# slp-rl/aero

Hardware: NVIDIA H100
Metric: audio-seconds/sec forward (higher is better)
Workload: dtype f16 tensor-core operands and activation storage (10-bit mantissa = tf32), fp32 accumulate / norm inputs / cell state

## Files before the change

aero_b200/cabi.py:

```python
from __future__ import annotations

import ctypes as C
import os

_HERE = os.path.dirname(os.path.abspath(__file__))
LIB_PATH = os.path.join(_HERE, "libaero_b200.so")

i32, i64, f32 = C.c_int32, C.c_int64, C.c_float
vp = C.c_void_p


class StftParams(C.Structure):
    _fields_ = [("n_fft", i32), ("hop", i32), ("win", i32), ("n_signals", i32), ("channels", i32),
                ("length", i32), ("frames", i32), ("bins_out", i32),
                ("z_stride_b", i64), ("z_stride_c", i64), ("z_stride_k", i64), ("z_stride_t", i64),
                ("flags", i32), ("reserved", i32)]


class IstftParams(C.Structure):
    _fields_ = [("n_fft", i32), ("hop", i32), ("win", i32), ("n_signals", i32), ("channels", i32),
                ("frames", i32), ("bins_in", i32), ("out_len", i32),
                ("z_stride_b", i64), ("z_stride_c", i64), ("z_stride_k", i64), ("z_stride_t", i64),
                ("flags", i32), ("reserved", i32)]

# ... 34 lines not shown

class ResampleParams(C.Structure):
    _fields_ = [("B", i32), ("C", i32), ("L_in", i32), ("orig", i32), ("up", i32), ("width", i32), ("taps", i32),
                ("L_hr", i32), ("L_valid", i32), ("halo", i32), ("fill", i32), ("normalize", i32), ("floor_", f32)]


ABI_VERSION = 3
TAPS_CONV, TAPS_CONVT, TAPS_MIX = 0, 1, 2
ACT_NONE, ACT_GELU, ACT_RELU, ACT_LEAKY, ACT_TANH = 0, 1, 2, 3, 4
TG_ROUND_TF32, TG_A_F16, TG_OUT_F16, TG_REVERSE = 1, 2, 4, 8
NA_NONE, NA_GELU, NA_GLU, NA_SNAKE, NA_GLU_SCALE_RES, NA_RELU, NA_LEAKY, NA_TANH = 0, 1, 2, 3, 4, 5, 6, 7
NA_NO_NORM = 16
STFT_ZERO_PAD, STFT_ADJ_SCALE, ISTFT_RAW = 1, 2, 1

SYMBOLS = {
    "aero_abi_version": (C.c_int, []),
    "aero_last_error": (C.c_char_p, []),
    "aero_device_arch": (C.c_int, []),
    "aero_launch_count": (C.c_uint64, []),
    "aero_stft_fwd": (C.c_int, [vp, vp, vp, vp, C.POINTER(StftParams), vp]),
    "aero_istft_fwd": (C.c_int, [vp, vp, vp, C.POINTER(IstftParams), vp]),
    "aero_tapgemm_fwd": (C.c_int, [vp] * 10 + [C.POINTER(TapGemmParams), vp]),
    "aero_tapgemm_tc_eligible": (C.c_int, [C.POINTER(TapGemmParams)]),
    "aero_sample_norm_fwd": (C.c_int, [vp, vp, vp, vp, i32, i64, i64, i32, vp]),
    "aero_norm_act_fwd": (C.c_int, [vp] * 8 + [C.POINTER(NormActParams), vp]),
    "aero_ftb_lin_out_fwd": (C.c_int, [vp] * 7 + [C.POINTER(FtbLinParams), vp]),
    "aero_ftb_lin_squeeze_fwd": (C.c_int, [vp, vp, vp, vp, i32, C.POINTER(FtbLinParams), vp]),
    "aero_freq_mix_small_fwd": (C.c_int, [vp, vp, vp, vp, i32, i32, i64, i32, vp]),
    "aero_lstm_rec_fwd": (C.c_int, [vp, vp, vp, vp, C.POINTER(LstmParams), vp]),
    "aero_local_attn_fwd": (C.c_int, [vp, vp, C.POINTER(AttnParams), vp]),
    "aero_lsd_fwd": (C.c_int, [vp, vp, vp, i32, i32, i32, i32, vp]),
    "aero_stft_loss_fwd": (C.c_int, [vp, vp, vp, i32, i32, i32, i32, vp]),
    "aero_stft_loss_bwd": (C.c_int, [vp, vp, vp, vp, i32, i32, i32, i32, f32, f32, vp]),
    "aero_tapgemm_wgrad": (C.c_int, [vp, vp, vp, vp, C.POINTER(TapGemmParams), i64, i64, i64, vp]),
    "aero_colsum": (C.c_int, [vp, vp, vp, vp, i32, i32, i64, i64, i64, i64, i32, i64, i64, vp]),
    "aero_add": (C.c_int, [vp, vp, i64, f32, vp]),
    "aero_add_f64": (C.c_int, [vp, vp, i64, vp]),
    "aero_gram": (C.c_int, [vp, vp, vp, vp, i32, i32, i64, i64, i64, i64, vp]),
    "aero_bcast_add": (C.c_int, [vp, vp, i32, i32, i32, i32, vp]),
    "aero_scale_rows": (C.c_int, [vp, vp, vp, i32, i64, i32, vp]),
    "aero_norm_act_train_fwd": (C.c_int, [vp] * 8 + [C.POINTER(NormActParams), vp]),
    "aero_norm_act_train_bwd": (C.c_int, [vp] * 13 + [i32, C.POINTER(NormActParams), vp]),
    "aero_adam_step": (C.c_int, [vp, i32, f32, f32, f32, f32, i32, f32, vp]),
    "aero_pack_kmajor_tf32": (C.c_int, [vp, vp, vp, i32, i32, i32, vp]),
    "aero_split_tf32": (C.c_int, [vp, vp, vp, i64, vp]),
    "aero_tapgemm_wgrad_tc_eligible": (C.c_int, [C.POINTER(TapGemmParams), vp, vp, vp]),
# ... 57 lines not shown
```

aero_b200/csrc/tapgemm_tc.cu:

```cuda
#include <cuda.h>
#include <mutex>
#include <unordered_map>
#include <string>
#include <cstring>
#include <cstdlib>

#include "tapgemm.cuh"
#include "tc_common.cuh"

namespace aero {

KernelFn tapgemm_tc_kernels_bn32(bool f16a, bool f16o, int amode, bool res, bool stats);
KernelFn tapgemm_tc_kernels_bn64(bool f16a, bool f16o, int amode, bool res, bool stats);
KernelFn tapgemm_tc_kernels_bn96(bool f16a, bool f16o, int amode, bool res, bool stats);
KernelFn tapgemm_tc_kernels_bn128(bool f16a, bool f16o, int amode, bool res, bool stats);

typedef CUresult (*EncodeTiledFn)(CUtensorMap*, CUtensorMapDataType, cuuint32_t, void*, const cuuint64_t*, const cuuint64_t*,
                                  const cuuint32_t*, const cuuint32_t*, CUtensorMapInterleave, CUtensorMapSwizzle,
                                  CUtensorMapL2promotion, CUtensorMapFloatOOBfill);

static EncodeTiledFn get_encode() {
    static EncodeTiledFn fn = nullptr;
    static std::once_flag once;
    std::call_once(once, [] {
        void* p = nullptr;
        cudaDriverEntryPointQueryResult qres;
        if (cudaGetDriverEntryPoint("cuTensorMapEncodeTiled", &p, cudaEnableDefault, &qres) == cudaSuccess &&
            qres == cudaDriverEntryPointSuccess)
            fn = reinterpret_cast<EncodeTiledFn>(p);
    });
    return fn;
}

struct MapKey {
    const void* base;
    uint64_t d[4], s[3];
    uint32_t box[4], rank, swz, pad_;
    bool operator==(const MapKey& o) const { return std::memcmp(this, &o, sizeof(MapKey)) == 0; }
// ... 67 lines not shown
        return p.w_sb == 0 && p.C1 % q == 0 && p.C2 == 0 && p.a1_st % q == 0 && p.a1_sb % q == 0 && p.N >= 8 &&
               p.stats_mode == 0 && !p.glu && p.F_out == 1 && p.F_in == 1 && tc_stages(p.N, pick_bn(p.N)) >= 2;
    if (p.w_sb != 0) return false;
    if (p.act == AERO_ACT_TANH) return false;
    if (p.act == AERO_ACT_LEAKY && (p.stats_mode != 0 || p.r_sb != 0 || p.r_sf != 0 || p.r_st != 0))
        return false;
    if (tc_stages(p.N, pick_bn(p.N)) < 2) return false;
    if (p.N < 8) return false;
    const int K = p.C1 + p.C2;
    if (K < 8 || (p.C1 % q) || (p.C2 % q)) return false;
    auto ok_strides = [q](int64_t sb, int64_t sf, int64_t st) { return sb % q == 0 && sf % q == 0 && st % q == 0 && st > 0; };
    if (p.C1 && !ok_strides(p.a1_sb, p.a1_sf, p.a1_st)) return false;
    if (p.C2 && !ok_strides(p.a2_sb, p.a2_sf, p.a2_st)) return false;
    if (p.stats_mode == 1) {
        const int Nout = p.glu ? p.N / 2 : p.N;
        if (p.groups < 1 || Nout % p.groups) return false;
        const int gw = Nout / p.groups;
        const int bn = pick_bn(p.N);
        if (gw % 8 || (p.glu ? bn / 2 : bn) / gw + 2 > 8) return false;
    }
    return true;
}

static int make_a_map(CUtensorMap* m, const void* base, int C, const aero_tapgemm_params& p, int64_t sb, int64_t sf, int64_t st, int esz) {
    uint64_t dims[4] = {(uint64_t)C, (uint64_t)p.T_in, (uint64_t)p.F_in, (uint64_t)p.B};
    int64_t s1 = st, s2 = sf, s3 = sb;
    if (s2 <= 0) s2 = s1 * p.T_in;
    if (s3 <= 0) s3 = s2 * p.F_in;
    uint64_t strides[3] = {(uint64_t)s1 * esz, (uint64_t)s2 * esz, (uint64_t)s3 * esz};
    uint32_t box[4] = {(uint32_t)(128 / esz), (uint32_t)kBM, 1, 1};
    return encode_map(m, base, 4, dims, strides, box, 0, esz);
}

struct TcKnobs {
    int direct_f32 = -1, direct_f16 = -1, stages = -1;
    TcKnobs() {
        auto rd = [](const char* name, int& v) { if (const char* e = getenv(name)) v = atoi(e); };
        rd("AERO_TC_DIRECT_F32", direct_f32); rd("AERO_TC_DIRECT_F16", direct_f16); rd("AERO_TC_STAGES", stages);
    }
};
static const TcKnobs& knobs() { static const TcKnobs k; return k; }

int tapgemm_tc_launch(const TapGemmArgs& g0, cudaStream_t st) {
    const TcKnobs& kn = knobs();
    TapGemmArgs g = g0;
    const aero_tapgemm_params& p = g.p;
    const bool f16a = p.precision == 2, f16o = (p.flags & AERO_TG_OUT_F16) != 0;
    const int esz = f16a ? 2 : 4, kBKc = 128 / esz;
    const int K = p.C1 + p.C2;
    const int BN = pick_bn(p.N);
    const int nslab = (p.mode == AERO_TAPS_CONVT) ? p.kf : p.kf * p.kt;
    CUtensorMap mA1, mA2, mW;
    int rc;
    const bool mix = p.mode == AERO_TAPS_MIX;
    if (mix) {
        uint64_t dims[3] = {(uint64_t)p.T, (uint64_t)p.C1, (uint64_t)p.B};
        uint64_t strides[2] = {(uint64_t)p.a1_st * esz, (uint64_t)(p.a1_sb > 0 ? p.a1_sb : (int64_t)p.a1_st * p.C1) * esz};
        uint32_t box[3] = {(uint32_t)(f16a ? 64 : 32), (uint32_t)kBKc, 1};
        if ((rc = encode_map(&mA1, g.a1, 3, dims, strides, box, 0, esz)) != AERO_OK) return rc;
    } else if (p.C1) { if ((rc = make_a_map(&mA1, g.a1, p.C1, p, p.a1_sb, p.a1_sf, p.a1_st, esz)) != AERO_OK) return rc; }
    if (p.C2) { if ((rc = make_a_map(&mA2, g.a2, p.C2, p, p.a2_sb, p.a2_sf, p.a2_st, esz)) != AERO_OK) return rc; }
    if (!p.C1) mA1 = mA2;
    if (!p.C2) mA2 = mA1;
    {
        const uint64_t npad = (uint64_t)((p.N + 3) & ~3);
        const uint64_t kp = f16a ? (uint64_t)((K + 7) & ~7) : (uint64_t)K;
        uint64_t dims[3] = {(uint64_t)K, npad, (uint64_t)nslab};
        uint64_t strides[2] = {kp * esz, kp * npad * esz};
        uint32_t box[3] = {(uint32_t)kBKc, (uint32_t)BN, 1};
        if ((rc = encode_map(&mW, g.w, 3, dims, strides, box, 0, esz)) != AERO_OK) return rc;
    }
    g.tiles_t = cdiv(p.T, kBM);
    g.direct_f32 = 0;
    g.direct_f16 = 2;
    if (kn.direct_f32 >= 0) g.direct_f32 = kn.direct_f32;
    if (kn.direct_f16 >= 0) g.direct_f16 = kn.direct_f16;
    const int64_t tiles = (int64_t)p.B * p.F_out * g.tiles_t;
    if (tiles > 2147483647LL) { set_error("aero_tapgemm_fwd: too many tiles"); return AERO_ERR_INVALID; }
    {
        const uint32_t divs[3] = {(uint32_t)cdiv(p.N, BN), (uint32_t)g.tiles_t, (uint32_t)p.F_out};
        for (int i = 0; i < 3; ++i) {
            uint32_t s = 0;
            while ((1ull << s) < divs[i]) ++s;
            const uint64_t two = 1ull << (31 + s);
            g.dv_mul[i] = (uint32_t)((two + divs[i] - 1) / divs[i]);
            g.dv_shr[i] = 31 + s;
        }
    }
    const int stage_bytes = kATileBytes + BN * 128;
    const int fixed = tc_fixed_smem(p.N, BN);
    int kStages = tc_stages(p.N, BN);
    if (kStages < 2) {
        set_error("aero_tapgemm_fwd(wgmma): N = %d leaves no shared memory for the pipeline", p.N);
        return AERO_ERR_UNSUPPORTED;
    }
    if (kn.stages >= 2 && kn.stages < kStages) kStages = kn.stages;
    const size_t smem = (size_t)kStages * stage_bytes + fixed;
    const int amode = p.glu ? 3 : (p.act == AERO_ACT_LEAKY ? 4 : p.act);
    if (p.glu && p.act != AERO_ACT_NONE) { set_error("aero_tapgemm_fwd(wgmma): GLU with an activation is not supported"); return AERO_ERR_UNSUPPORTED; }
    const bool res = g.residual != nullptr, stats = p.stats_mode != 0;
    const KernelFn kern = BN == 32 ? tapgemm_tc_kernels_bn32(f16a, f16o, amode, res, stats)
                        : BN == 64 ? tapgemm_tc_kernels_bn64(f16a, f16o, amode, res, stats)
                        : BN == 96 ? tapgemm_tc_kernels_bn96(f16a, f16o, amode, res, stats)
                                   : tapgemm_tc_kernels_bn128(f16a, f16o, amode, res, stats);
    if (!kern) {
        set_error("aero_tapgemm_fwd(wgmma): epilogue (act %d, residual %d, stats %d) is not built for operands %s / outputs %s",
                  amode, (int)res, (int)stats, f16a ? "f16" : "tf32", f16o ? "f16" : "f32");
        return AERO_ERR_UNSUPPORTED;
    }
    cudaFuncSetAttribute(kern, cudaFuncAttributeMaxDynamicSharedMemorySize, 227 * 1024);
    static int num_sms = 0;
    if (num_sms == 0) {
        int dev = 0;
        cudaGetDevice(&dev);
        cudaDeviceGetAttribute(&num_sms, cudaDevAttrMultiProcessorCount, dev);
    }
    const int n_tiles = cdiv(p.N, BN);
    const int64_t tiles_total = tiles * n_tiles;
    if (tiles_total > 2147483647LL) { set_error("aero_tapgemm_fwd: too many tiles"); return AERO_ERR_INVALID; }
    const int64_t want = num_sms;
    g.last_tile = (int)tiles_total - 1;
    dim3 grid((unsigned)(tiles_total < want ? tiles_total : want));
    kern<<<grid, kThreads, smem, st>>>(mA1, mA2, mW, g, kStages, n_tiles, (int)tiles_total);
    return check_launch("aero_tapgemm_fwd(wgmma)");
}

}
```

aero_b200/csrc/tapgemm_tc_bn128.cu:

```cuda
#include "tapgemm_tc_kernel.cuh"

namespace aero {
KernelFn tapgemm_tc_kernels_bn128(bool f16a, bool f16o, int amode, bool res, bool stats) { return pick_kernel_bn<128>(f16a, f16o, amode, res, stats); }
}
```

aero_b200/csrc/tapgemm_tc_bn32.cu:

```cuda
#include "tapgemm_tc_kernel.cuh"

namespace aero {
KernelFn tapgemm_tc_kernels_bn32(bool f16a, bool f16o, int amode, bool res, bool stats) { return pick_kernel_bn<32>(f16a, f16o, amode, res, stats); }
}
```

aero_b200/csrc/tapgemm_tc_bn64.cu:

```cuda
#include "tapgemm_tc_kernel.cuh"

namespace aero {
KernelFn tapgemm_tc_kernels_bn64(bool f16a, bool f16o, int amode, bool res, bool stats) { return pick_kernel_bn<64>(f16a, f16o, amode, res, stats); }
}
```

aero_b200/csrc/tapgemm_tc_bn96.cu:

```cuda
#include "tapgemm_tc_kernel.cuh"

namespace aero {
KernelFn tapgemm_tc_kernels_bn96(bool f16a, bool f16o, int amode, bool res, bool stats) { return pick_kernel_bn<96>(f16a, f16o, amode, res, stats); }
}
```

aero_b200/csrc/tapgemm_tc_kernel.cuh:

```cuda
#pragma once
#include <cuda.h>
#include <type_traits>

#include "tapgemm.cuh"
#include "tc_common.cuh"


namespace aero {

template <bool F16A> struct OperandKind { static constexpr int kBK = F16A ? 64 : 32; };

struct TapIter {
    int fi, dt, slab;
};
__device__ __forceinline__ bool tap_geometry(const aero_tapgemm_params& p, int tap, int fo, TapIter& it) {
    if (p.mode == AERO_TAPS_CONV) {
        const int jf = tap / p.kt, jt = tap - jf * p.kt;
        it.fi = fo * p.stride_f + jf - p.pad_f;
        it.dt = jt * p.dil_t - p.pad_t;
        it.slab = tap;
    } else {
        const int fof = fo + p.f_out_offset;
        it.fi = fof / p.stride_f - tap;
        it.dt = 0;
        it.slab = fof % p.stride_f + tap * p.stride_f;
    }
    return it.fi >= 0 && it.fi < p.F_in;
}

struct TileCoord {
    int b, fo, t0, n0, n_iters;
};
__device__ __forceinline__ int fast_div(int n, uint32_t mul, uint32_t shr) {
    return (int)(((uint64_t)(uint32_t)n * mul) >> shr);
}
__device__ __forceinline__ int valid_taps(const aero_tapgemm_params& p, int fo, int ntaps) {
    if (p.mode == AERO_TAPS_CONV) {
        const int base = fo * p.stride_f - p.pad_f;
        const int lo = max(0, -base), hi = min(p.kf - 1, p.F_in - 1 - base);
        return max(0, hi - lo + 1) * p.kt;
    }
    const int a = (fo + p.f_out_offset) / p.stride_f;
    const int lo = max(0, a - p.F_in + 1), hi = min(ntaps - 1, a);
    return max(0, hi - lo + 1);
}
__device__ __forceinline__ TileCoord tile_coord(const TapGemmArgs& g, int tile, int n_tiles, int BN, int nch1, int nch2) {
    const aero_tapgemm_params& p = g.p;
    TileCoord c;
    if (p.flags & AERO_TG_REVERSE) tile = g.last_tile - tile;
    const int mt = fast_div(tile, g.dv_mul[0], g.dv_shr[0]), nt = tile - mt * n_tiles;
    const int row = fast_div(mt, g.dv_mul[1], g.dv_shr[1]), tt = mt - row * g.tiles_t;
    c.b = fast_div(row, g.dv_mul[2], g.dv_shr[2]);
    c.fo = row - c.b * p.F_out;
    c.t0 = tt * kBM;
    c.n0 = nt * BN;
    c.n_iters = (p.mode == AERO_TAPS_MIX) ? nch1 : valid_taps(p, c.fo, g.ntaps) * (nch1 + nch2);
    return c;
}

template <int AMODE>
__device__ __forceinline__ void epilogue_stage_a(const uint32_t (&r)[16], uint32_t stg_row, uint32_t sbias) {
    float4 bv[4];
#pragma unroll
    for (int j = 0; j < 4; ++j) bv[j] = lds128(sbias + 16 * j);
#pragma unroll
    for (int j = 0; j < 16; j += 4) {
        float v[4] = {__uint_as_float(r[j]) + bv[j / 4].x, __uint_as_float(r[j + 1]) + bv[j / 4].y,
                      __uint_as_float(r[j + 2]) + bv[j / 4].z, __uint_as_float(r[j + 3]) + bv[j / 4].w};
#pragma unroll
        for (int u = 0; u < 4; ++u) {
            if (AMODE == 1) v[u] = gelu_exact(v[u]);
// ... 195 lines not shown
                if (j < n_ok) {
                    const int gi = (no0 + j) / gw;
                    if (gi != cur_g) {
                        if (cur_g >= 0) {
                            const float a = warp_sum(ssum), c = warp_sum(ssq);
                            if (lane == 0) { sh->stats[ew][cur_g - g_lo][0] += a; sh->stats[ew][cur_g - g_lo][1] += c; }
                        }
                        cur_g = gi; ssum = 0.f; ssq = 0.f;
                    }
                    if (row_ok) {
                        ssum += (o[j] + o[j + 1]) + (o[j + 2] + o[j + 3]);
                        ssq += (o[j] * o[j] + o[j + 1] * o[j + 1]) + (o[j + 2] * o[j + 2] + o[j + 3] * o[j + 3]);
                    }
                }
            }
        }
    }
    if (STATS && cur_g >= 0) {
        const float a = warp_sum(ssum), c = warp_sum(ssq);
        if (lane == 0) { sh->stats[ew][cur_g - g_lo][0] += a; sh->stats[ew][cur_g - g_lo][1] += c; }
    }
}

template <int BN, bool F16A>
__device__ __forceinline__ void tile_mainloop(TcShared* sh, uint8_t* smem, int& stage, uint32_t& phase, const int kStages, const int stage_bytes,
                                              const int n_iters, const bool mix, const int wg, float* acc, const int ldacc) {
    float d[BN / 2];
    const int tid = threadIdx.x & 127, wl = tid >> 5, lane = tid & 31;
    int prev = -1;
    for (int i = 0; i < n_iters; ++i) {
        mbar_wait(&sh->full[stage], phase);
        const uint32_t sa = smem_u32(smem + stage * stage_bytes);
        const uint64_t db = make_desc_sw128(sa + kATileBytes);
        wgmma_fence();
        if (mix && F16A) {
            if constexpr (F16A) {
                const uint32_t sw = sa + (uint32_t)wg * 8192u;
                const uint64_t da = (uint64_t)((sw >> 4) & 0x3FFF) | ((uint64_t)(8192 >> 4) << 16) | ((uint64_t)(1024 >> 4) << 32) | ((uint64_t)1 << 62);
#pragma unroll
                for (int k = 0; k < 4; ++k) Wgmma<BN, true, 1>::ss(d, da + (uint64_t)(k * (2048 >> 4)), db + 2 * k, (i > 0 || k > 0) ? 1u : 0u);
            }
        } else if (mix) {
            if constexpr (!F16A) {
                const int m = wg * 64 + wl * 16 + (lane >> 2), c = lane & 3;
#pragma unroll
                for (int k = 0; k < 4; ++k) {
                    uint32_t a[4];
#pragma unroll
                    for (int u = 0; u < 4; ++u) {
                        const int mm = m + (u & 1) * 8, kk = 8 * k + c + (u >> 1) * 4;
                        const uint32_t addr = sa + (uint32_t)((mm >> 5) * 4096 + kk * 128 + ((((mm & 31) >> 2) ^ (kk & 7)) << 4) + ((mm & 3) << 2));
                        asm volatile("ld.shared.b32 %0, [%1];" : "=r"(a[u]) : "r"(addr));
                    }
                    Wgmma<BN, false, 0>::rs(d, a, db + 2 * k, (i > 0 || k > 0) ? 1u : 0u);
                }
            }
        } else {
            const uint64_t da = make_desc_sw128(sa + (uint32_t)wg * (64 * 128));
#pragma unroll
            for (int k = 0; k < 4; ++k)
                Wgmma<BN, F16A, 0>::ss(d, da + 2 * k, db + 2 * k, (i > 0 || k > 0) ? 1u : 0u);
        }
        wgmma_commit();
        wgmma_wait<1>();
        if (prev >= 0 && tid == 0) mbar_arrive(&sh->empty[prev]);
        prev = stage;
        if (++stage == kStages) { stage = 0; phase ^= 1; }
    }
    wgmma_wait<0>();
    if (prev >= 0 && tid == 0) mbar_arrive(&sh->empty[prev]);
    float* row = acc + (wg * 64 + wl * 16 + (lane >> 2)) * ldacc + 2 * (lane & 3);
#pragma unroll
    for (int j = 0; j < BN / 8; ++j) {
        *reinterpret_cast<float2*>(row + 8 * j) = make_float2(d[4 * j], d[4 * j + 1]);
        *reinterpret_cast<float2*>(row + 8 * ldacc + 8 * j) = make_float2(d[4 * j + 2], d[4 * j + 3]);
    }
}

template <int BN, int AMODE, bool RES, bool STATS, bool F16A, bool F16O>
__global__ void __launch_bounds__(kThreads, 1)
tapgemm_tc_kernel(const __grid_constant__ CUtensorMap mapA1, const __grid_constant__ CUtensorMap mapA2,
                  const __grid_constant__ CUtensorMap mapW, const TapGemmArgs g, const int kStages, const int n_tiles,
                  const int tiles_total) {
    extern __shared__ uint8_t smem_raw[];
    uint8_t* smem = reinterpret_cast<uint8_t*>((reinterpret_cast<uintptr_t>(smem_raw) + 1023) & ~(uintptr_t)1023);
    constexpr int stage_bytes = kATileBytes + BN * 128;
    TcShared* sh = reinterpret_cast<TcShared*>(smem + kStages * stage_bytes);
    float* const sbias_f = reinterpret_cast<float*>(sh + 1);
    const uint32_t sbias = smem_u32(sbias_f);
    float* const acc = sbias_f + n_tiles * BN;
    constexpr int ldacc = BN + 4;

    using TO = typename std::conditional<F16O, __half, float>::type;
    constexpr int kBKc = OperandKind<F16A>::kBK;
    const aero_tapgemm_params& p = g.p;
    const int warp = threadIdx.x >> 5, lane = threadIdx.x & 31;
    const int nch1 = (p.C1 + kBKc - 1) / kBKc, nch2 = (p.C2 + kBKc - 1) / kBKc;
    const bool mix = p.mode == AERO_TAPS_MIX;

    for (int i = threadIdx.x; i < n_tiles * BN; i += kThreads) sbias_f[i] = (g.bias && i < g.p.N) ? g.bias[i] : 0.f;
    if (threadIdx.x == 0) {
        for (int s = 0; s < kStages; ++s) { mbar_init(&sh->full[s], 1); mbar_init(&sh->empty[s], 2); }
        asm volatile("fence.mbarrier_init.release.cluster;" ::: "memory");
        for (int w = 0; w < kEpiWarps; ++w)
            for (int i = 0; i < 8; ++i) { sh->stats[w][i][0] = 0.f; sh->stats[w][i][1] = 0.f; }
    }
    __syncthreads();

    if (warp == 0) {
        if (lane == 0) {
            asm volatile("prefetch.tensormap [%0];" ::"l"(&mapA1) : "memory");
            asm volatile("prefetch.tensormap [%0];" ::"l"(&mapW) : "memory");
            int stage = 0;
            uint32_t phase = 0;
            const uint32_t tx = (uint32_t)stage_bytes;
            int ptl = 0;
            for (int tile = blockIdx.x; tile < tiles_total; tile += gridDim.x, ++ptl) {
                const TileCoord c = tile_coord(g, tile, n_tiles, BN, nch1, nch2);
                if (mix) {
                    for (int kc = 0; kc < nch1; ++kc) {
                        mbar_wait(&sh->empty[stage], phase ^ 1);
                        uint8_t* sa = smem + stage * stage_bytes;
                        mbar_expect_tx(&sh->full[stage], tx);
                        constexpr int kBoxM = F16A ? 64 : 32;
#pragma unroll
                        for (int j = 0; j < 128 / kBoxM; ++j)
                            tma_load_3d(sa + j * (kATileBytes / (128 / kBoxM)), &mapA1, &sh->full[stage], c.t0 + kBoxM * j, kc * kBKc, c.b);
                        tma_load_3d(sa + kATileBytes, &mapW, &sh->full[stage], kc * kBKc, c.n0, 0);
                        if (++stage == kStages) { stage = 0; phase ^= 1; }
                    }
                    continue;
                }
                for (int tap = 0; tap < g.ntaps; ++tap) {
                    TapIter it;
                    if (!tap_geometry(p, tap, c.fo, it)) continue;
                    for (int src = 0; src < 2; ++src) {
                        const int nch = src ? nch2 : nch1;
                        const CUtensorMap* mA = src ? &mapA2 : &mapA1;
                        const int kw0 = src ? p.C1 : 0;
                        for (int kc = 0; kc < nch; ++kc) {
                            mbar_wait(&sh->empty[stage], phase ^ 1);
                            uint8_t* sa = smem + stage * stage_bytes;
                            mbar_expect_tx(&sh->full[stage], tx);
                            tma_load_4d(sa, mA, &sh->full[stage], kc * kBKc, c.t0 + it.dt, it.fi, c.b);
                            tma_load_3d(sa + kATileBytes, &mapW, &sh->full[stage], kw0 + kc * kBKc, c.n0, it.slab);
                            if (++stage == kStages) { stage = 0; phase ^= 1; }
                        }
                    }
                }
            }
        }
    } else if (warp >= 4) {
        const int wg = (warp >> 2) - 1;
        const int ew = warp - 4;
        const int q = 2 * wg + (warp & 1);
        const int grp = (warp >> 1) & 1;
        const int m = q * 32 + lane;
        const int Nout = p.glu ? p.N / 2 : p.N;
        const int gw = (p.stats_mode == 1) ? Nout / p.groups : Nout;
        const bool rnd = (p.flags & 1) && !F16O;
        const int c_start = grp * 16, c_step = 32;
        const bool fast = !mix && g.vec_o && !g.colscale && (p.stats_mode == 0 || gw % 4 == 0);
        int stage = 0, local = 0;
        uint32_t phase = 0;
        for (int tile = blockIdx.x; tile < tiles_total; tile += gridDim.x, ++local) {
            const TileCoord tc = tile_coord(g, tile, n_tiles, BN, nch1, nch2);
            const int b = tc.b, fo = tc.fo, t0 = tc.t0, n0 = tc.n0, n_iters = tc.n_iters;
            tile_mainloop<BN, F16A>(sh, smem, stage, phase, kStages, stage_bytes, n_iters, mix, wg, acc, ldacc);
            warpgroup_sync(1 + wg);
            const uint32_t tacc = smem_u32(acc + m * ldacc);
            const int t = t0 + m;
            const bool row_ok = t < p.T;
            float sa = 1.f, sb = 0.f;
            if (g.samp_affine) { sa = g.samp_affine[2 * b]; sb = g.samp_affine[2 * b + 1]; }
            TO* op = static_cast<TO*>(g.out) + (int64_t)b * p.o_sb + (int64_t)fo * p.o_sf + (int64_t)t * p.o_st;
            const TO* rp = g.residual ? static_cast<const TO*>(g.residual) + (int64_t)b * p.r_sb + (int64_t)fo * p.r_sf + (int64_t)t * p.r_st : nullptr;
            const float* csp = g.colscale ? g.colscale + (int64_t)b * p.cs_sb + (int64_t)t * p.cs_st : nullptr;
            const float* adp = g.addend_fn ? g.addend_fn + (int64_t)fo * Nout : nullptr;
            int cur_g = -1;
            float ssum = 0.f, ssq = 0.f;
            const int g_lo = (p.glu ? n0 >> 1 : n0) / gw;

            if (mix) {
                const float gate = (row_ok && g.colscale) ? g.colscale[(int64_t)b * p.cs_sb + t] : 1.f;
                TO* ob = static_cast<TO*>(g.out) + (int64_t)b * p.o_sb + t;
                for (int c0 = c_start; c0 < BN; c0 += c_step) {
                    uint32_t r[16];
                    acc_ld16(tacc + 4u * (uint32_t)c0, r);
                    if (row_ok) {
#pragma unroll
                        for (int j = 0; j < 16; ++j) {
// ... 89 lines not shown
                    const float a = warp_sum(ssum), c = warp_sum(ssq);
                    if (lane == 0) { sh->stats[ew][cur_g - g_lo][0] = a; sh->stats[ew][cur_g - g_lo][1] = c; }
                }
            }
            warpgroup_sync(1 + wg);
            if (p.stats_mode != 0) {
                __syncwarp();
                if (lane < 8) {
                    const float a = sh->stats[ew][lane][0], c = sh->stats[ew][lane][1];
                    const int gi = g_lo + lane;
                    const int ngroups = (p.stats_mode == 1) ? p.groups : 1;
                    if (gi < ngroups && (a != 0.f || c != 0.f)) {
                        const int64_t slot = (p.stats_mode == 1) ? ((int64_t)b * p.groups + gi) : ((int64_t)b * p.F_out + fo);
                        atomicAdd(&g.stats[2 * slot], (double)a);
                        atomicAdd(&g.stats[2 * slot + 1], (double)c);
                    }
                    sh->stats[ew][lane][0] = 0.f;
                    sh->stats[ew][lane][1] = 0.f;
                }
                __syncwarp();
            }
        }
    }
}



template <int BN, bool F16A, bool F16O>
static KernelFn pick_kernel(int amode, bool res, bool stats) {
#define AERO_TC_K(A, R, S) tapgemm_tc_kernel<BN, A, R, S, F16A, F16O>
    if (amode == 4) return (res || stats) ? nullptr : AERO_TC_K(4, false, false);
    if constexpr (!F16A && !F16O) {
        static const KernelFn table[4][2][2] = {
            {{AERO_TC_K(0, false, false), AERO_TC_K(0, false, true)}, {AERO_TC_K(0, true, false), AERO_TC_K(0, true, true)}},
            {{AERO_TC_K(1, false, false), AERO_TC_K(1, false, true)}, {AERO_TC_K(1, true, false), AERO_TC_K(1, true, true)}},
            {{AERO_TC_K(2, false, false), AERO_TC_K(2, false, true)}, {AERO_TC_K(2, true, false), AERO_TC_K(2, true, true)}},
            {{AERO_TC_K(3, false, false), AERO_TC_K(3, false, true)}, {AERO_TC_K(3, true, false), AERO_TC_K(3, true, true)}}};
        return table[amode][res][stats];
    } else if constexpr (F16O) {
        if (stats) return (amode == 0 && !res) ? AERO_TC_K(0, false, true) : nullptr;
        if (res) return amode == 0 ? AERO_TC_K(0, true, false) : nullptr;
        switch (amode) {
            case 0: return AERO_TC_K(0, false, false);
            case 1: return AERO_TC_K(1, false, false);
            case 2: return AERO_TC_K(2, false, false);
            default: return AERO_TC_K(3, false, false);
        }
    } else {
        if (res) return nullptr;
        if (stats) return amode == 0 ? AERO_TC_K(0, false, true) : nullptr;
        switch (amode) {
            case 0: return AERO_TC_K(0, false, false);
            case 1: return AERO_TC_K(1, false, false);
            case 2: return AERO_TC_K(2, false, false);
            default: return AERO_TC_K(3, false, false);
        }
    }
#undef AERO_TC_K
}

template <int BN>
static KernelFn pick_kernel_bn(bool f16a, bool f16o, int amode, bool res, bool stats) {
    return f16a ? (f16o ? pick_kernel<BN, true, true>(amode, res, stats) : pick_kernel<BN, true, false>(amode, res, stats))
                : (f16o ? pick_kernel<BN, false, true>(amode, res, stats) : pick_kernel<BN, false, false>(amode, res, stats));
}

}
```

aero_b200/csrc/tc_common.cuh:

```cuda
#pragma once
#include <cuda.h>
#include "common.cuh"
#include "wgmma.cuh"

namespace aero {

int encode_map(CUtensorMap* out, const void* base, uint32_t rank, const uint64_t* dims, const uint64_t* strides_bytes,
               const uint32_t* box, int swizzle_mode = 0, int elem_bytes = 4);

__device__ __forceinline__ uint32_t smem_u32(const void* p) { return (uint32_t)__cvta_generic_to_shared(p); }

__device__ __forceinline__ void mbar_init(uint64_t* bar, uint32_t count) {
    asm volatile("mbarrier.init.shared::cta.b64 [%0], %1;" ::"r"(smem_u32(bar)), "r"(count));
}
__device__ __forceinline__ void mbar_expect_tx(uint64_t* bar, uint32_t bytes) {
    asm volatile("mbarrier.arrive.expect_tx.shared::cta.b64 _, [%0], %1;" ::"r"(smem_u32(bar)), "r"(bytes) : "memory");
}
__device__ __forceinline__ bool mbar_try_wait(uint64_t* bar, uint32_t parity) {
    uint32_t ok;
    asm volatile(
        "{\n\t.reg .pred p;\n\t"
        "mbarrier.try_wait.parity.shared::cta.b64 p, [%1], %2;\n\t"
        "selp.u32 %0, 1, 0, p;\n\t}"
        : "=r"(ok)
        : "r"(smem_u32(bar)), "r"(parity)
        : "memory");
    return ok != 0;
}
__device__ __forceinline__ void mbar_wait(uint64_t* bar, uint32_t parity) {
    for (uint32_t spin = 0; !mbar_try_wait(bar, parity); ++spin) {
        if (spin > (1u << 24)) asm volatile("trap;");
    }
}
__device__ __forceinline__ void tma_load_4d(void* dst, const CUtensorMap* map, uint64_t* bar, int c0, int c1, int c2, int c3) {
    asm volatile(
        "cp.async.bulk.tensor.4d.shared::cluster.global.tile.mbarrier::complete_tx::bytes [%0], [%1, {%3, %4, %5, %6}], [%2];"
        ::"r"(smem_u32(dst)), "l"(map), "r"(smem_u32(bar)), "r"(c0), "r"(c1), "r"(c2), "r"(c3)
        : "memory");
}
__device__ __forceinline__ void tma_load_3d(void* dst, const CUtensorMap* map, uint64_t* bar, int c0, int c1, int c2) {
    asm volatile(
        "cp.async.bulk.tensor.3d.shared::cluster.global.tile.mbarrier::complete_tx::bytes [%0], [%1, {%3, %4, %5}], [%2];"
        ::"r"(smem_u32(dst)), "l"(map), "r"(smem_u32(bar)), "r"(c0), "r"(c1), "r"(c2)
        : "memory");
}
__device__ __forceinline__ void tma_load_2d(void* dst, const CUtensorMap* map, uint64_t* bar, int c0, int c1) {
    asm volatile(
        "cp.async.bulk.tensor.2d.shared::cluster.global.tile.mbarrier::complete_tx::bytes [%0], [%1, {%3, %4}], [%2];"
        ::"r"(smem_u32(dst)), "l"(map), "r"(smem_u32(bar)), "r"(c0), "r"(c1)
        : "memory");
}
__device__ __forceinline__ float4 lds128(uint32_t saddr) {
    float4 v;
    asm volatile("ld.shared.v4.f32 {%0, %1, %2, %3}, [%4];" : "=f"(v.x), "=f"(v.y), "=f"(v.z), "=f"(v.w) : "r"(saddr));
    return v;
}
__device__ __forceinline__ void sts128(uint32_t saddr, float4 v) {
    asm volatile("st.shared.v4.f32 [%0], {%1, %2, %3, %4};" ::"r"(saddr), "f"(v.x), "f"(v.y), "f"(v.z), "f"(v.w) : "memory");
}
__device__ __forceinline__ void sts64(uint32_t saddr, float a, float b) {
    asm volatile("st.shared.v2.f32 [%0], {%1, %2};" ::"r"(saddr), "f"(a), "f"(b) : "memory");
}
__device__ __forceinline__ void acc_ld16(uint32_t saddr, uint32_t (&r)[16]) {
#pragma unroll
    for (int j = 0; j < 4; ++j) {
        const float4 v = lds128(saddr + 16u * j);
        r[4 * j] = __float_as_uint(v.x); r[4 * j + 1] = __float_as_uint(v.y); r[4 * j + 2] = __float_as_uint(v.z); r[4 * j + 3] = __float_as_uint(v.w);
    }
}
__device__ __forceinline__ void warpgroup_sync(int id) { asm volatile("bar.sync %0, 128;" ::"r"(id) : "memory"); }
__device__ __forceinline__ void mbar_arrive(uint64_t* bar) {
    asm volatile("mbarrier.arrive.shared::cta.b64 _, [%0];" ::"r"(smem_u32(bar)) : "memory");
}
__device__ __forceinline__ void fence_proxy_async_smem() { asm volatile("fence.proxy.async.shared::cta;" ::: "memory"); }

}
```

include/aero_b200.h:

```cpp
#ifndef AERO_B200_H
#define AERO_B200_H

#include <stddef.h>
#include <stdint.h>

#ifdef __cplusplus
extern "C" {
#endif

typedef void* aero_stream_t;

enum aero_status {
    AERO_OK = 0,
    AERO_ERR_INVALID = -1,
    AERO_ERR_UNSUPPORTED = -2,
    AERO_ERR_LAUNCH = -3,
    AERO_ERR_NO_DEVICE = -4
};

int aero_abi_version(void);
const char* aero_last_error(void);
int aero_device_arch(void);
uint64_t aero_launch_count(void);

// ... 36 lines not shown
    int32_t C1, C2;
    int32_t mode, kf, kt, stride_f, pad_f, dil_t, pad_t, f_out_offset;
    int32_t act, glu, stats_mode, groups;
    int64_t a1_sb, a1_sf, a1_st;
    int64_t a2_sb, a2_sf, a2_st;
    int64_t w_sb;
    int64_t o_sb, o_sf, o_st;
    int64_t r_sb, r_sf, r_st;
    int64_t cs_sb, cs_st;
    int32_t precision;
    int32_t flags;
} aero_tapgemm_params;
enum {
    AERO_TG_ROUND_TF32 = 1,
    AERO_TG_A_F16 = 2,
    AERO_TG_OUT_F16 = 4,
    AERO_TG_REVERSE = 8
};
int aero_tapgemm_fwd(const void* a1, const void* a2, const void* w, const float* bias,
                     const float* addend_fn, const float* colscale, const void* residual,
                     const float* samp_affine, void* out, double* stats,
                     const aero_tapgemm_params* p, aero_stream_t stream);
int aero_tapgemm_tc_eligible(const aero_tapgemm_params* p);

int aero_sample_norm_fwd(const float* x, const double* stats, float* y, float* samp_affine,
                         int32_t B, int64_t count, int64_t extent, int32_t round_tf32, aero_stream_t stream);

enum { AERO_NA_NONE = 0, AERO_NA_GELU = 1, AERO_NA_GLU = 2, AERO_NA_SNAKE = 3, AERO_NA_GLU_SCALE_RES = 4,
       AERO_NA_RELU = 5, AERO_NA_LEAKY = 6 , AERO_NA_TANH = 7  };
enum { AERO_NA_NO_NORM = 16 };
typedef struct {
    int32_t B, F_in, F_out, f_off, T, C;
    int32_t groups, scope, op;
    float eps;
    int32_t flags;
} aero_norm_act_params;
int aero_norm_act_fwd(const void* x, const double* stats, const float* gamma, const float* beta,
                      const float* snake_a, const float* scale, const void* residual, void* y,
                      const aero_norm_act_params* p, aero_stream_t stream);

typedef struct {
    int32_t B, F, T, N, J;
    int32_t flags;
    int64_t z_sb, z_sf, zm_sb, zm_sf;
} aero_ftb_lin_params;
int aero_ftb_lin_out_fwd(const float* z, const float* zm, const float* M, const float* s, const float* V, const float* d,
// ... 120 lines not shown
```

Measured before the change: 3338.

## Pair CTAs in clusters and multicast shared weight tiles via TMA

For f16 2D convolutions (kf>1, kt>1) with an even number of time tiles, the tap-GEMM kernel now launches in 2-CTA clusters. Each cluster handles two adjacent time tiles that share the same weight tile. Each CTA loads half of that weight tile with TMA multicast to both CTAs, which is meant to halve weight-operand L2/global traffic. The cost is cross-CTA empty-barrier arrivals, cluster syncs and occupancy-limited cluster scheduling, which can add lockstep stalls between the paired CTAs.

```diff
diff --git a/aero_b200/cabi.py b/aero_b200/cabi.py
--- a/aero_b200/cabi.py
+++ b/aero_b200/cabi.py
@@ -80,6 +80,8 @@
     "aero_istft_fwd": (C.c_int, [vp, vp, vp, C.POINTER(IstftParams), vp]),
     "aero_tapgemm_fwd": (C.c_int, [vp] * 10 + [C.POINTER(TapGemmParams), vp]),
     "aero_tapgemm_tc_eligible": (C.c_int, [C.POINTER(TapGemmParams)]),
+    "aero_tapgemm_tc_cluster": (C.c_int, [C.POINTER(TapGemmParams)]),
+    "aero_tapgemm_tc_paired_launches": (C.c_uint64, []),
     "aero_sample_norm_fwd": (C.c_int, [vp, vp, vp, vp, i32, i64, i64, i32, vp]),
     "aero_norm_act_fwd": (C.c_int, [vp] * 8 + [C.POINTER(NormActParams), vp]),
     "aero_ftb_lin_out_fwd": (C.c_int, [vp] * 7 + [C.POINTER(FtbLinParams), vp]),
diff --git a/aero_b200/csrc/tapgemm_tc.cu b/aero_b200/csrc/tapgemm_tc.cu
--- a/aero_b200/csrc/tapgemm_tc.cu
+++ b/aero_b200/csrc/tapgemm_tc.cu
@@ -1,4 +1,6 @@
 #include <cuda.h>
+#include <atomic>
+#include <map>
 #include <mutex>
 #include <unordered_map>
 #include <string>
@@ -10,10 +12,10 @@
 
 namespace aero {
 
-KernelFn tapgemm_tc_kernels_bn32(bool f16a, bool f16o, int amode, bool res, bool stats);
-KernelFn tapgemm_tc_kernels_bn64(bool f16a, bool f16o, int amode, bool res, bool stats);
-KernelFn tapgemm_tc_kernels_bn96(bool f16a, bool f16o, int amode, bool res, bool stats);
-KernelFn tapgemm_tc_kernels_bn128(bool f16a, bool f16o, int amode, bool res, bool stats);
+KernelFn tapgemm_tc_kernels_bn32(bool f16a, bool f16o, int amode, bool res, bool stats, bool pair);
+KernelFn tapgemm_tc_kernels_bn64(bool f16a, bool f16o, int amode, bool res, bool stats, bool pair);
+KernelFn tapgemm_tc_kernels_bn96(bool f16a, bool f16o, int amode, bool res, bool stats, bool pair);
+KernelFn tapgemm_tc_kernels_bn128(bool f16a, bool f16o, int amode, bool res, bool stats, bool pair);
 
 typedef CUresult (*EncodeTiledFn)(CUtensorMap*, CUtensorMapDataType, cuuint32_t, void*, const cuuint64_t*, const cuuint64_t*,
                                   const cuuint32_t*, const cuuint32_t*, CUtensorMapInterleave, CUtensorMapSwizzle,
@@ -127,6 +129,35 @@
     return true;
 }
 
+bool tapgemm_tc_paired(const aero_tapgemm_params& p) {
+    return p.precision == 2 && p.mode == AERO_TAPS_CONV && p.kf > 1 && p.kt > 1 && cdiv(p.T, kBM) % 2 == 0;
+}
+static std::atomic<uint64_t> g_paired_launches{0};
+
+static int max_active_pairs(KernelFn kern, size_t smem) {
+    static std::mutex mu;
+    static std::map<std::pair<const void*, size_t>, int> cache;
+    const auto key = std::make_pair(reinterpret_cast<const void*>(kern), smem);
+    std::lock_guard<std::mutex> lk(mu);
+    auto it = cache.find(key);
+    if (it != cache.end()) return it->second;
+    int dev = 0, sms = 0, n = 0;
+    cudaGetDevice(&dev);
+    cudaDeviceGetAttribute(&sms, cudaDevAttrMultiProcessorCount, dev);
+    cudaLaunchAttribute at;
+    at.id = cudaLaunchAttributeClusterDimension;
+    at.val.clusterDim.x = 2; at.val.clusterDim.y = 1; at.val.clusterDim.z = 1;
+    cudaLaunchConfig_t cfg = {};
+    cfg.gridDim = dim3((unsigned)(2 * sms));
+    cfg.blockDim = dim3(kThreads);
+    cfg.dynamicSmemBytes = smem;
+    cfg.attrs = &at;
+    cfg.numAttrs = 1;
+    if (cudaOccupancyMaxActiveClusters(&n, reinterpret_cast<const void*>(kern), &cfg) != cudaSuccess) { cudaGetLastError(); n = 0; }
+    if (n > 0) cache.emplace(key, n);
+    return n;
+}
+
 static int make_a_map(CUtensorMap* m, const void* base, int C, const aero_tapgemm_params& p, int64_t sb, int64_t sf, int64_t st, int esz) {
     uint64_t dims[4] = {(uint64_t)C, (uint64_t)p.T_in, (uint64_t)p.F_in, (uint64_t)p.B};
     int64_t s1 = st, s2 = sf, s3 = sb;
@@ -155,6 +186,7 @@
     const int K = p.C1 + p.C2;
     const int BN = pick_bn(p.N);
     const int nslab = (p.mode == AERO_TAPS_CONVT) ? p.kf : p.kf * p.kt;
+    const bool pair = tapgemm_tc_paired(p);
     CUtensorMap mA1, mA2, mW;
     int rc;
     const bool mix = p.mode == AERO_TAPS_MIX;
@@ -172,7 +204,7 @@
         const uint64_t kp = f16a ? (uint64_t)((K + 7) & ~7) : (uint64_t)K;
         uint64_t dims[3] = {(uint64_t)K, npad, (uint64_t)nslab};
         uint64_t strides[2] = {kp * esz, kp * npad * esz};
-        uint32_t box[3] = {(uint32_t)kBKc, (uint32_t)BN, 1};
+        uint32_t box[3] = {(uint32_t)kBKc, (uint32_t)(pair ? BN / 2 : BN), 1};
         if ((rc = encode_map(&mW, g.w, 3, dims, strides, box, 0, esz)) != AERO_OK) return rc;
     }
     g.tiles_t = cdiv(p.T, kBM);
@@ -204,10 +236,10 @@
     const int amode = p.glu ? 3 : (p.act == AERO_ACT_LEAKY ? 4 : p.act);
     if (p.glu && p.act != AERO_ACT_NONE) { set_error("aero_tapgemm_fwd(wgmma): GLU with an activation is not supported"); return AERO_ERR_UNSUPPORTED; }
     const bool res = g.residual != nullptr, stats = p.stats_mode != 0;
-    const KernelFn kern = BN == 32 ? tapgemm_tc_kernels_bn32(f16a, f16o, amode, res, stats)
-                        : BN == 64 ? tapgemm_tc_kernels_bn64(f16a, f16o, amode, res, stats)
-                        : BN == 96 ? tapgemm_tc_kernels_bn96(f16a, f16o, amode, res, stats)
-                                   : tapgemm_tc_kernels_bn128(f16a, f16o, amode, res, stats);
+    const KernelFn kern = BN == 32 ? tapgemm_tc_kernels_bn32(f16a, f16o, amode, res, stats, pair)
+                        : BN == 64 ? tapgemm_tc_kernels_bn64(f16a, f16o, amode, res, stats, pair)
+                        : BN == 96 ? tapgemm_tc_kernels_bn96(f16a, f16o, amode, res, stats, pair)
+                                   : tapgemm_tc_kernels_bn128(f16a, f16o, amode, res, stats, pair);
     if (!kern) {
         set_error("aero_tapgemm_fwd(wgmma): epilogue (act %d, residual %d, stats %d) is not built for operands %s / outputs %s",
                   amode, (int)res, (int)stats, f16a ? "f16" : "tf32", f16o ? "f16" : "f32");
@@ -223,11 +255,38 @@
     const int n_tiles = cdiv(p.N, BN);
     const int64_t tiles_total = tiles * n_tiles;
     if (tiles_total > 2147483647LL) { set_error("aero_tapgemm_fwd: too many tiles"); return AERO_ERR_INVALID; }
-    const int64_t want = num_sms;
     g.last_tile = (int)tiles_total - 1;
-    dim3 grid((unsigned)(tiles_total < want ? tiles_total : want));
-    kern<<<grid, kThreads, smem, st>>>(mA1, mA2, mW, g, kStages, n_tiles, (int)tiles_total);
-    return check_launch("aero_tapgemm_fwd(wgmma)");
-}
-
-}
+    if (!pair) {
+        const int64_t want = num_sms;
+        dim3 grid((unsigned)(tiles_total < want ? tiles_total : want));
+        kern<<<grid, kThreads, smem, st>>>(mA1, mA2, mW, g, kStages, n_tiles, (int)tiles_total);
+        return check_launch("aero_tapgemm_fwd(wgmma)");
+    }
+    const int pairs = max_active_pairs(kern, smem);
+    if (pairs < 1) {
+        set_error("aero_tapgemm_fwd(wgmma): no 2-CTA cluster fits with %zu bytes of shared memory", smem);
+        return AERO_ERR_LAUNCH;
+    }
+    const int64_t units = tiles_total / 2;
+    cudaLaunchAttribute at;
+    at.id = cudaLaunchAttributeClusterDimension;
+    at.val.clusterDim.x = 2; at.val.clusterDim.y = 1; at.val.clusterDim.z = 1;
+    cudaLaunchConfig_t cfg = {};
+    cfg.gridDim = dim3((unsigned)(2 * (units < pairs ? units : pairs)));
+    cfg.blockDim = dim3(kThreads);
+    cfg.dynamicSmemBytes = smem;
+    cfg.stream = st;
+    cfg.attrs = &at;
+    cfg.numAttrs = 1;
+    const cudaError_t e = cudaLaunchKernelEx(&cfg, kern, mA1, mA2, mW, g, kStages, n_tiles, (int)tiles_total);
+    const int rc2 = check_launch("aero_tapgemm_fwd(wgmma, paired)");
+    if (rc2 != AERO_OK) return rc2;
+    if (e != cudaSuccess) { set_error("aero_tapgemm_fwd(wgmma, paired): %s", cudaGetErrorString(e)); return AERO_ERR_LAUNCH; }
+    g_paired_launches.fetch_add(1, std::memory_order_relaxed);
+    return AERO_OK;
+}
+
+}
+
+extern "C" int aero_tapgemm_tc_cluster(const aero_tapgemm_params* p) { return p && aero::tapgemm_tc_paired(*p) ? 2 : 1; }
+extern "C" uint64_t aero_tapgemm_tc_paired_launches(void) { return aero::g_paired_launches.load(); }
diff --git a/aero_b200/csrc/tapgemm_tc_bn128.cu b/aero_b200/csrc/tapgemm_tc_bn128.cu
--- a/aero_b200/csrc/tapgemm_tc_bn128.cu
+++ b/aero_b200/csrc/tapgemm_tc_bn128.cu
@@ -1,5 +1,7 @@
 #include "tapgemm_tc_kernel.cuh"
 
 namespace aero {
-KernelFn tapgemm_tc_kernels_bn128(bool f16a, bool f16o, int amode, bool res, bool stats) { return pick_kernel_bn<128>(f16a, f16o, amode, res, stats); }
+KernelFn tapgemm_tc_kernels_bn128(bool f16a, bool f16o, int amode, bool res, bool stats, bool pair) {
+    return pick_kernel_bn<128>(f16a, f16o, amode, res, stats, pair);
 }
+}
diff --git a/aero_b200/csrc/tapgemm_tc_bn32.cu b/aero_b200/csrc/tapgemm_tc_bn32.cu
--- a/aero_b200/csrc/tapgemm_tc_bn32.cu
+++ b/aero_b200/csrc/tapgemm_tc_bn32.cu
@@ -1,5 +1,7 @@
 #include "tapgemm_tc_kernel.cuh"
 
 namespace aero {
-KernelFn tapgemm_tc_kernels_bn32(bool f16a, bool f16o, int amode, bool res, bool stats) { return pick_kernel_bn<32>(f16a, f16o, amode, res, stats); }
+KernelFn tapgemm_tc_kernels_bn32(bool f16a, bool f16o, int amode, bool res, bool stats, bool pair) {
+    return pick_kernel_bn<32>(f16a, f16o, amode, res, stats, pair);
 }
+}
diff --git a/aero_b200/csrc/tapgemm_tc_bn64.cu b/aero_b200/csrc/tapgemm_tc_bn64.cu
--- a/aero_b200/csrc/tapgemm_tc_bn64.cu
+++ b/aero_b200/csrc/tapgemm_tc_bn64.cu
@@ -1,5 +1,7 @@
 #include "tapgemm_tc_kernel.cuh"
 
 namespace aero {
-KernelFn tapgemm_tc_kernels_bn64(bool f16a, bool f16o, int amode, bool res, bool stats) { return pick_kernel_bn<64>(f16a, f16o, amode, res, stats); }
+KernelFn tapgemm_tc_kernels_bn64(bool f16a, bool f16o, int amode, bool res, bool stats, bool pair) {
+    return pick_kernel_bn<64>(f16a, f16o, amode, res, stats, pair);
 }
+}
diff --git a/aero_b200/csrc/tapgemm_tc_bn96.cu b/aero_b200/csrc/tapgemm_tc_bn96.cu
--- a/aero_b200/csrc/tapgemm_tc_bn96.cu
+++ b/aero_b200/csrc/tapgemm_tc_bn96.cu
@@ -1,5 +1,7 @@
 #include "tapgemm_tc_kernel.cuh"
 
 namespace aero {
-KernelFn tapgemm_tc_kernels_bn96(bool f16a, bool f16o, int amode, bool res, bool stats) { return pick_kernel_bn<96>(f16a, f16o, amode, res, stats); }
+KernelFn tapgemm_tc_kernels_bn96(bool f16a, bool f16o, int amode, bool res, bool stats, bool pair) {
+    return pick_kernel_bn<96>(f16a, f16o, amode, res, stats, pair);
 }
+}
diff --git a/aero_b200/csrc/tapgemm_tc_kernel.cuh b/aero_b200/csrc/tapgemm_tc_kernel.cuh
--- a/aero_b200/csrc/tapgemm_tc_kernel.cuh
+++ b/aero_b200/csrc/tapgemm_tc_kernel.cuh
@@ -44,9 +44,12 @@
     const int lo = max(0, a - p.F_in + 1), hi = min(ntaps - 1, a);
     return max(0, hi - lo + 1);
 }
-__device__ __forceinline__ TileCoord tile_coord(const TapGemmArgs& g, int tile, int n_tiles, int BN, int nch1, int nch2) {
+template <bool PAIR>
+__device__ __forceinline__ TileCoord tile_coord(const TapGemmArgs& g, int unit, uint32_t rank, int n_tiles, int BN, int nch1, int nch2) {
     const aero_tapgemm_params& p = g.p;
     TileCoord c;
+    int tile = unit;
+    if (PAIR) tile += (fast_div(unit, g.dv_mul[0], g.dv_shr[0]) + (int)rank) * n_tiles;
     if (p.flags & AERO_TG_REVERSE) tile = g.last_tile - tile;
     const int mt = fast_div(tile, g.dv_mul[0], g.dv_shr[0]), nt = tile - mt * n_tiles;
     const int row = fast_div(mt, g.dv_mul[1], g.dv_shr[1]), tt = mt - row * g.tiles_t;
@@ -288,11 +291,18 @@
     }
 }
 
-template <int BN, bool F16A>
+template <int BN, bool F16A, bool PAIR>
 __device__ __forceinline__ void tile_mainloop(TcShared* sh, uint8_t* smem, int& stage, uint32_t& phase, const int kStages, const int stage_bytes,
-                                              const int n_iters, const bool mix, const int wg, float* acc, const int ldacc) {
+                                              const int n_iters, const bool mix, const int wg, float* acc, const int ldacc,
+                                              const uint32_t peer) {
     float d[BN / 2];
     const int tid = threadIdx.x & 127, wl = tid >> 5, lane = tid & 31;
+    auto release = [&](int s) {
+        if (tid == 0) {
+            mbar_arrive(&sh->empty[s]);
+            if (PAIR) mbar_arrive_cluster(&sh->empty[s], peer);
+        }
+    };
     int prev = -1;
     for (int i = 0; i < n_iters; ++i) {
         mbar_wait(&sh->full[stage], phase);
@@ -329,12 +339,12 @@
         }
         wgmma_commit();
         wgmma_wait<1>();
-        if (prev >= 0 && tid == 0) mbar_arrive(&sh->empty[prev]);
+        if (prev >= 0) release(prev);
         prev = stage;
         if (++stage == kStages) { stage = 0; phase ^= 1; }
     }
     wgmma_wait<0>();
-    if (prev >= 0 && tid == 0) mbar_arrive(&sh->empty[prev]);
+    if (prev >= 0) release(prev);
     float* row = acc + (wg * 64 + wl * 16 + (lane >> 2)) * ldacc + 2 * (lane & 3);
 #pragma unroll
     for (int j = 0; j < BN / 8; ++j) {
@@ -343,7 +353,7 @@
     }
 }
 
-template <int BN, int AMODE, bool RES, bool STATS, bool F16A, bool F16O>
+template <int BN, int AMODE, bool RES, bool STATS, bool F16A, bool F16O, bool PAIR>
 __global__ void __launch_bounds__(kThreads, 1)
 tapgemm_tc_kernel(const __grid_constant__ CUtensorMap mapA1, const __grid_constant__ CUtensorMap mapA2,
                   const __grid_constant__ CUtensorMap mapW, const TapGemmArgs g, const int kStages, const int n_tiles,
@@ -363,15 +373,20 @@
     const int warp = threadIdx.x >> 5, lane = threadIdx.x & 31;
     const int nch1 = (p.C1 + kBKc - 1) / kBKc, nch2 = (p.C2 + kBKc - 1) / kBKc;
     const bool mix = p.mode == AERO_TAPS_MIX;
+    constexpr bool pair = PAIR;
+    const uint32_t rank = pair ? cluster_ctarank() : 0u, peer = rank ^ 1u;
+    const int unit0 = pair ? (int)(blockIdx.x >> 1) : (int)blockIdx.x, unit_step = pair ? (int)(gridDim.x >> 1) : (int)gridDim.x;
+    const int units = pair ? tiles_total >> 1 : tiles_total;
 
     for (int i = threadIdx.x; i < n_tiles * BN; i += kThreads) sbias_f[i] = (g.bias && i < g.p.N) ? g.bias[i] : 0.f;
     if (threadIdx.x == 0) {
-        for (int s = 0; s < kStages; ++s) { mbar_init(&sh->full[s], 1); mbar_init(&sh->empty[s], 2); }
+        for (int s = 0; s < kStages; ++s) { mbar_init(&sh->full[s], 1); mbar_init(&sh->empty[s], pair ? 4 : 2); }
         asm volatile("fence.mbarrier_init.release.cluster;" ::: "memory");
         for (int w = 0; w < kEpiWarps; ++w)
             for (int i = 0; i < 8; ++i) { sh->stats[w][i][0] = 0.f; sh->stats[w][i][1] = 0.f; }
     }
     __syncthreads();
+    if (pair) cluster_sync();
 
     if (warp == 0) {
         if (lane == 0) {
@@ -380,9 +395,13 @@
             int stage = 0;
             uint32_t phase = 0;
             const uint32_t tx = (uint32_t)stage_bytes;
-            int ptl = 0;
-            for (int tile = blockIdx.x; tile < tiles_total; tile += gridDim.x, ++ptl) {
-                const TileCoord c = tile_coord(g, tile, n_tiles, BN, nch1, nch2);
+            const int b_row = pair ? (int)rank * (BN / 2) : 0;
+            auto load_b = [&](uint8_t* sa, int k, int n0, int slab) {
+                if (pair) tma_load_3d_multicast(sa + kATileBytes + b_row * 128, &mapW, &sh->full[stage], k, n0 + b_row, slab, (uint16_t)3);
+                else tma_load_3d(sa + kATileBytes, &mapW, &sh->full[stage], k, n0, slab);
+            };
+            for (int unit = unit0; unit < units; unit += unit_step) {
+                const TileCoord c = tile_coord<PAIR>(g, unit, rank, n_tiles, BN, nch1, nch2);
                 if (mix) {
                     for (int kc = 0; kc < nch1; ++kc) {
                         mbar_wait(&sh->empty[stage], phase ^ 1);
@@ -392,7 +411,7 @@
 #pragma unroll
                         for (int j = 0; j < 128 / kBoxM; ++j)
                             tma_load_3d(sa + j * (kATileBytes / (128 / kBoxM)), &mapA1, &sh->full[stage], c.t0 + kBoxM * j, kc * kBKc, c.b);
-                        tma_load_3d(sa + kATileBytes, &mapW, &sh->full[stage], kc * kBKc, c.n0, 0);
+                        load_b(sa, kc * kBKc, c.n0, 0);
                         if (++stage == kStages) { stage = 0; phase ^= 1; }
                     }
                     continue;
@@ -409,7 +428,7 @@
                             uint8_t* sa = smem + stage * stage_bytes;
                             mbar_expect_tx(&sh->full[stage], tx);
                             tma_load_4d(sa, mA, &sh->full[stage], kc * kBKc, c.t0 + it.dt, it.fi, c.b);
-                            tma_load_3d(sa + kATileBytes, &mapW, &sh->full[stage], kw0 + kc * kBKc, c.n0, it.slab);
+                            load_b(sa, kw0 + kc * kBKc, c.n0, it.slab);
                             if (++stage == kStages) { stage = 0; phase ^= 1; }
                         }
                     }
@@ -427,12 +446,12 @@
         const bool rnd = (p.flags & 1) && !F16O;
         const int c_start = grp * 16, c_step = 32;
         const bool fast = !mix && g.vec_o && !g.colscale && (p.stats_mode == 0 || gw % 4 == 0);
-        int stage = 0, local = 0;
+        int stage = 0;
         uint32_t phase = 0;
-        for (int tile = blockIdx.x; tile < tiles_total; tile += gridDim.x, ++local) {
-            const TileCoord tc = tile_coord(g, tile, n_tiles, BN, nch1, nch2);
+        for (int unit = unit0; unit < units; unit += unit_step) {
+            const TileCoord tc = tile_coord<PAIR>(g, unit, rank, n_tiles, BN, nch1, nch2);
             const int b = tc.b, fo = tc.fo, t0 = tc.t0, n0 = tc.n0, n_iters = tc.n_iters;
-            tile_mainloop<BN, F16A>(sh, smem, stage, phase, kStages, stage_bytes, n_iters, mix, wg, acc, ldacc);
+            tile_mainloop<BN, F16A, PAIR>(sh, smem, stage, phase, kStages, stage_bytes, n_iters, mix, wg, acc, ldacc, peer);
             warpgroup_sync(1 + wg);
             const uint32_t tacc = smem_u32(acc + m * ldacc);
             const int t = t0 + m;
@@ -568,20 +587,32 @@
             }
         }
     }
-}
-
-
+    if (pair) cluster_sync();
+}
+
+
+
+template <int BN, int AMODE, bool RES, bool STATS, bool F16A, bool F16O>
+static KernelFn kernel_of(bool pair) {
+    if constexpr (F16A) {
+        if (pair) return tapgemm_tc_kernel<BN, AMODE, RES, STATS, F16A, F16O, true>;
+    }
+    return pair ? nullptr : tapgemm_tc_kernel<BN, AMODE, RES, STATS, F16A, F16O, false>;
+}
 
 template <int BN, bool F16A, bool F16O>
-static KernelFn pick_kernel(int amode, bool res, bool stats) {
-#define AERO_TC_K(A, R, S) tapgemm_tc_kernel<BN, A, R, S, F16A, F16O>
+static KernelFn pick_kernel(int amode, bool res, bool stats, bool pair) {
+#define AERO_TC_K(A, R, S) kernel_of<BN, A, R, S, F16A, F16O>(pair)
     if (amode == 4) return (res || stats) ? nullptr : AERO_TC_K(4, false, false);
     if constexpr (!F16A && !F16O) {
+        if (pair) return nullptr;
+#define AERO_TC_K1(A, R, S) tapgemm_tc_kernel<BN, A, R, S, F16A, F16O, false>
         static const KernelFn table[4][2][2] = {
-            {{AERO_TC_K(0, false, false), AERO_TC_K(0, false, true)}, {AERO_TC_K(0, true, false), AERO_TC_K(0, true, true)}},
-            {{AERO_TC_K(1, false, false), AERO_TC_K(1, false, true)}, {AERO_TC_K(1, true, false), AERO_TC_K(1, true, true)}},
-            {{AERO_TC_K(2, false, false), AERO_TC_K(2, false, true)}, {AERO_TC_K(2, true, false), AERO_TC_K(2, true, true)}},
-            {{AERO_TC_K(3, false, false), AERO_TC_K(3, false, true)}, {AERO_TC_K(3, true, false), AERO_TC_K(3, true, true)}}};
+            {{AERO_TC_K1(0, false, false), AERO_TC_K1(0, false, true)}, {AERO_TC_K1(0, true, false), AERO_TC_K1(0, true, true)}},
+            {{AERO_TC_K1(1, false, false), AERO_TC_K1(1, false, true)}, {AERO_TC_K1(1, true, false), AERO_TC_K1(1, true, true)}},
+            {{AERO_TC_K1(2, false, false), AERO_TC_K1(2, false, true)}, {AERO_TC_K1(2, true, false), AERO_TC_K1(2, true, true)}},
+            {{AERO_TC_K1(3, false, false), AERO_TC_K1(3, false, true)}, {AERO_TC_K1(3, true, false), AERO_TC_K1(3, true, true)}}};
+#undef AERO_TC_K1
         return table[amode][res][stats];
     } else if constexpr (F16O) {
         if (stats) return (amode == 0 && !res) ? AERO_TC_K(0, false, true) : nullptr;
@@ -606,9 +637,9 @@
 }
 
 template <int BN>
-static KernelFn pick_kernel_bn(bool f16a, bool f16o, int amode, bool res, bool stats) {
-    return f16a ? (f16o ? pick_kernel<BN, true, true>(amode, res, stats) : pick_kernel<BN, true, false>(amode, res, stats))
-                : (f16o ? pick_kernel<BN, false, true>(amode, res, stats) : pick_kernel<BN, false, false>(amode, res, stats));
-}
-
-}
+static KernelFn pick_kernel_bn(bool f16a, bool f16o, int amode, bool res, bool stats, bool pair) {
+    return f16a ? (f16o ? pick_kernel<BN, true, true>(amode, res, stats, pair) : pick_kernel<BN, true, false>(amode, res, stats, pair))
+                : (f16o ? pick_kernel<BN, false, true>(amode, res, stats, pair) : pick_kernel<BN, false, false>(amode, res, stats, pair));
+}
+
+}
diff --git a/aero_b200/csrc/tc_common.cuh b/aero_b200/csrc/tc_common.cuh
--- a/aero_b200/csrc/tc_common.cuh
+++ b/aero_b200/csrc/tc_common.cuh
@@ -44,6 +44,14 @@
         ::"r"(smem_u32(dst)), "l"(map), "r"(smem_u32(bar)), "r"(c0), "r"(c1), "r"(c2)
         : "memory");
 }
+__device__ __forceinline__ void tma_load_3d_multicast(void* dst, const CUtensorMap* map, uint64_t* bar, int c0, int c1, int c2,
+                                                      uint16_t cta_mask) {
+    asm volatile(
+        "cp.async.bulk.tensor.3d.shared::cluster.global.tile.mbarrier::complete_tx::bytes.multicast::cluster"
+        " [%0], [%1, {%4, %5, %6}], [%2], %3;"
+        ::"r"(smem_u32(dst)), "l"(map), "r"(smem_u32(bar)), "h"(cta_mask), "r"(c0), "r"(c1), "r"(c2)
+        : "memory");
+}
 __device__ __forceinline__ void tma_load_2d(void* dst, const CUtensorMap* map, uint64_t* bar, int c0, int c1) {
     asm volatile(
         "cp.async.bulk.tensor.2d.shared::cluster.global.tile.mbarrier::complete_tx::bytes [%0], [%1, {%3, %4}], [%2];"
@@ -74,4 +82,18 @@
 }
 __device__ __forceinline__ void fence_proxy_async_smem() { asm volatile("fence.proxy.async.shared::cta;" ::: "memory"); }
 
+__device__ __forceinline__ uint32_t cluster_ctarank() {
+    uint32_t r;
+    asm volatile("mov.u32 %0, %%cluster_ctarank;" : "=r"(r));
+    return r;
 }
+__device__ __forceinline__ void mbar_arrive_cluster(uint64_t* bar, uint32_t cta) {
+    uint32_t remote;
+    asm volatile("mapa.shared::cluster.u32 %0, %1, %2;" : "=r"(remote) : "r"(smem_u32(bar)), "r"(cta));
+    asm volatile("mbarrier.arrive.shared::cluster.b64 _, [%0];" ::"r"(remote) : "memory");
+}
+__device__ __forceinline__ void cluster_sync() {
+    asm volatile("barrier.cluster.arrive.release;\n\tbarrier.cluster.wait.acquire;" ::: "memory");
+}
+
+}
diff --git a/include/aero_b200.h b/include/aero_b200.h
--- a/include/aero_b200.h
+++ b/include/aero_b200.h
@@ -82,6 +82,8 @@
                      const float* samp_affine, void* out, double* stats,
                      const aero_tapgemm_params* p, aero_stream_t stream);
 int aero_tapgemm_tc_eligible(const aero_tapgemm_params* p);
+int aero_tapgemm_tc_cluster(const aero_tapgemm_params* p);
+uint64_t aero_tapgemm_tc_paired_launches(void);
 
 int aero_sample_norm_fwd(const float* x, const double* stats, float* y, float* samp_affine,
                          int32_t B, int64_t count, int64_t extent, int32_t round_tf32, aero_stream_t stream);
```

Result: faster. 3395, median of 6 (+1.7%).
